# Christovis/astrild

Hardware: AMD Instinct MI355X
Metric: particles/sec CIC+3D-FFT P(k) on 1024^3 grid (higher is better)
Workload: dtype f32

## Files before the change

astrild_amd/csrc/fft_tile.hip:

```cpp
#include "ast_common.h"
#include "fft_roots.h"
#include "lowk_sums.h"
#include "paint_tile_geom.h"
#include <algorithm>
#include <cmath>
#include <cstring>
#include <mutex>
#include <vector>

namespace {

__device__ constexpr float kCos32[16] = {
    1.0f, 0.9807852804032304f, 0.9238795325112867f, 0.8314696123025452f, 0.7071067811865476f,
    0.5555702330196023f, 0.38268343236508984f, 0.19509032201612833f, 0.0f, -0.1950903220161282f,
    -0.3826834323650897f, -0.555570233019602f, -0.7071067811865475f, -0.8314696123025453f,
    -0.9238795325112867f, -0.9807852804032304f};
__device__ constexpr float kSin32[16] = {
    0.0f, 0.19509032201612825f, 0.3826834323650898f, 0.5555702330196022f, 0.7071067811865475f,
    0.8314696123025452f, 0.9238795325112867f, 0.9807852804032304f, 1.0f, 0.9807852804032304f,
    0.9238795325112867f, 0.8314696123025455f, 0.7071067811865476f, 0.5555702330196022f,
    0.3826834323650899f, 0.1950903220161286f};

typedef float f2v __attribute__((ext_vector_type(2)));
template <bool NT>
// ... 29 lines not shown
                v[blk + j] = a + b;
                const cf2 d = a - b;
                const int t = j * (16 / h);
                if (t == 0) v[blk + j + h] = d;
                else if (t == 8) v[blk + j + h] = d.yx * cf2{1.0f, -1.0f};
                else v[blk + j + h] = cmul_cf(d, cf2{kCos32[t], -kSin32[t]});
            }
        }
    }
#pragma unroll
    for (int i = 0; i < R; ++i) vv[i] = from_cf(v[i]);
}

__device__ inline int tile_isqrt(int v) {
    return (int)__builtin_amdgcn_sqrtf((float)v + 0.5f);
}

__global__ void tile_isqrt_table_kernel(int* out, int count) {
    for (int v = blockIdx.x * blockDim.x + threadIdx.x; v < count; v += gridDim.x * blockDim.x) out[v] = tile_isqrt(v);
}

struct ShellMask { const float2* src; long long lo2, hi2; int ky0 = 0; int pass = 0;
                   size_t src_elem_stride = 0, src_batch_stride = 0;
                   int epi_skip = 0, no_nyq = 0; };

constexpr int SHELL_BATCH = 8;
#ifndef XPASS_ATOMICS
#define XPASS_ATOMICS 1
#endif
struct ShellBatch { int count = 0; float2* work[SHELL_BATCH]; long long lo2[SHELL_BATCH], hi2[SHELL_BATCH]; };
struct C2RBatch { int count = 0; const float2* in[SHELL_BATCH]; float* out[SHELL_BATCH]; int kmax[SHELL_BATCH]; };

struct DiscEntry { int offb; unsigned S, cumS, lohi; };
struct PackDst { float2* out = nullptr; unsigned c1_log2 = 0; unsigned nbatch = 0; float2* self_out = nullptr; unsigned self_part = ~0u; unsigned pitch = 0;
                 const DiscEntry* disc = nullptr; const unsigned short* gk = nullptr; unsigned part = 0;
                 unsigned xmajor = 0; };

template <int R1, int R2, int C, bool POWER, bool INV = false, int PACK = 0, bool TAB = false>
__global__ void __launch_bounds__(C * (R1 > R2 ? R1 : R2))
__attribute__((amdgpu_waves_per_eu((POWER || C > 16) && R1 * R2 >= 1024 ? 4 : 1, (POWER || C > 16) && R1 * R2 >= 1024 ? 4 : 8)))
strided_c2c_kernel(float2* __restrict__ data, const float2* __restrict__ tw_g, size_t elem_stride,
                   size_t ncols, size_t batch_stride, unsigned tiles_per_batch, float scale,
                   double* __restrict__ partial, const unsigned* __restrict__ edge_fall, ShellMask mask = ShellMask{nullptr, 0, 0},
                   PackDst pack = PackDst{}, ShellBatch sb = ShellBatch{}) {
    constexpr int N = R1 * R2;
    constexpr int NT = C * (R1 > R2 ? R1 : R2);
    constexpr int NB = N / 2 - 1;
    constexpr bool SPLIT = (POWER || C > 16) && R1 == R2 && N * C * sizeof(float2) > 64 * 1024;
    constexpr int YN = SPLIT ? N / 2 : N;
    extern __shared__ float2 lds[];
    float2* Y = lds;
    float2* tw = lds + YN * C;
    double* shell = reinterpret_cast<double*>(lds + YN * C + N);
    unsigned tile = blockIdx.x % tiles_per_batch, b = blockIdx.x / tiles_per_batch;
    if ((gridDim.x / tiles_per_batch) % 8u == 0u) {
        const unsigned xcd = blockIdx.x & 7u, slot = blockIdx.x >> 3;
        b = (slot / tiles_per_batch) * 8u + xcd;
        tile = slot % tiles_per_batch;
    }
    const size_t c0 = (size_t)tile * C;
    if (INV && sb.count > 0) {
        data = sb.work[blockIdx.y];
        mask.lo2 = sb.lo2[blockIdx.y];
        mask.hi2 = sb.hi2[blockIdx.y];
    }
    if (INV && mask.hi2 > 0) {
        const long long kb = (long long)((int)b > N / 2 ? (int)b - N : (int)b);
        const long long r2 = (long long)(c0 * c0) + (mask.pass == 0 ? kb * kb : 0);
        if (r2 >= mask.hi2) return;
    }
    const float2* disc_base = nullptr;
    unsigned disc_S = 0;
    int disc_ky = 0;
    if (!INV && POWER && pack.disc != nullptr) {
        const unsigned subb = b % R1, gk = pack.gk[pack.part * (pack.nbatch / R1) + b / R1];
        const DiscEntry e = pack.disc[(size_t)tile * R2 + gk];
        const unsigned lo = e.lohi & 255u, hi = (e.lohi >> 8) & 255u;
        if (subb - lo >= hi - lo) {
            for (int i = threadIdx.x; i < NB; i += NT) partial[((size_t)b * tiles_per_batch + tile) * NB + i] = 0.0;
            return;
        }
        disc_ky = (int)(gk * R1 + subb);
        if (pack.xmajor) {
            disc_base = data + ((long long)e.offb + (long long)(subb * 16u)) * (long long)pack.xmajor;
            disc_S = 16u;
        } else {
            disc_base = data + ((long long)e.offb + (long long)(subb * 16u));
            disc_S = e.S;
        }
    } else if (!INV && POWER && (mask.hi2 > 0 || mask.no_nyq)) {
        const long long kyi = (long long)b + mask.ky0, ky = kyi > N / 2 ? kyi - N : kyi;
        if ((mask.hi2 > 0 && ky * ky + (long long)(c0 * c0) > mask.hi2) || (mask.no_nyq && c0 >= (size_t)(N / 2))) {
            for (int i = threadIdx.x; i < NB; i += NT) partial[((size_t)b * tiles_per_batch + tile) * NB + i] = 0.0;
            return;
        }
    }
    for (int i = threadIdx.x; i < N; i += NT) tw[i] = tw_g[i];
    if (POWER)
        for (int i = threadIdx.x; i <= NB; i += NT) shell[i] = 0.0;
    const int c = threadIdx.x % C, sub = threadIdx.x / C;
    const bool col_ok = (unsigned)c0 + (unsigned)c < (unsigned)ncols;
    float2 u[R2];
    {
        const bool task1 = sub < R2;
        float2 v[R1];
        const bool own = INV && mask.src != nullptr && mask.src_elem_stride != 0;
        size_t es_in = own ? mask.src_elem_stride : elem_stride;
        const float2* ubase = (INV && mask.src ? mask.src : data) + (size_t)b * (own ? mask.src_batch_stride : batch_stride);
        const int lsub = task1 ? sub : R2 - 1;
        uint32_t voff = (uint32_t)lsub * (uint32_t)es_in + min((uint32_t)c0 + (uint32_t)c, (uint32_t)ncols - 1u);
        if (POWER && !INV && disc_base != nullptr) {
            es_in = disc_S;
            ubase = disc_base;
            voff = (uint32_t)lsub * disc_S + (uint32_t)c;
        }
        if (INV && mask.hi2 > 0 && mask.pass == 1) {
            const long long c02 = (long long)(c0 * c0);
#pragma unroll
            for (int n1 = 0; n1 < R1; ++n1) {
                const int row = n1 * R2 + lsub;
                const long long ky = row > N / 2 ? row - N : row;
                v[n1] = make_float2(0.f, 0.f);
                if (ky * ky + c02 < mask.hi2) v[n1] = (ubase + (size_t)(n1 * R2) * es_in)[voff];
            }
        } else if (INV && mask.hi2 > 0) {
            const long long kyb = (long long)((int)b > N / 2 ? (int)b - N : (int)b);
            const long long r2yz = kyb * kyb + (long long)(c0 * c0);
#pragma unroll
            for (int n1 = 0; n1 < R1; ++n1) {
                const int lo = n1 * R2, hi = lo + R2 - 1;
                const long long kxmin = hi <= N / 2 ? lo : (lo >= N / 2 ? N - hi : 0);
                v[n1] = make_float2(0.f, 0.f);
                if (kxmin * kxmin + r2yz < mask.hi2) v[n1] = (ubase + (size_t)(n1 * R2) * es_in)[voff];
            }
        } else {
#pragma unroll
            for (int n1 = 0; n1 < R1; ++n1) v[n1] = ld_stream<(!INV && N >= 1024)>(ubase + (size_t)(n1 * R2) * es_in + voff);
        }
        if (INV) {
            if (mask.hi2 > 0 && mask.pass == 0) {
                const long long kz = (long long)min(c0 + c, ncols - 1), ky = (long long)((int)b > N / 2 ? (int)b - N : (int)b);
                const long long m2yz = ky * ky + kz * kz;
#pragma unroll
                for (int n1 = 0; n1 < R1; ++n1) {
                    const int row = n1 * R2 + lsub;
                    const long long kx = row > N / 2 ? row - N : row, m2 = kx * kx + m2yz;
                    if (m2 < mask.lo2 || m2 >= mask.hi2) v[n1] = make_float2(0.f, 0.f);
                }
            }
#pragma unroll
            for (int n1 = 0; n1 < R1; ++n1) v[n1].y = -v[n1].y;
        }
        fft_reg<R1>(v);
        __syncthreads();
        if (!SPLIT) {
            if (task1) {
#pragma unroll
                for (int k1 = 0; k1 < R1; ++k1) {
                    float2 y = v[bitrev(k1, ilog2(R1))];
                    if (k1 != 0) y = cmul(y, tw[sub * k1]);
// ... 53 lines not shown
                const int offb = __builtin_amdgcn_readlane(ev.x, k2);
                const unsigned S = (unsigned)__builtin_amdgcn_readlane(ev.y, k2), cumS = (unsigned)__builtin_amdgcn_readlane(ev.z, k2);
                const unsigned lohi = (unsigned)__builtin_amdgcn_readlane(ev.w, k2);
                const unsigned lo = lohi & 255u, hi = (lohi >> 8) & 255u, part = lohi >> 16;
                if (pack.xmajor) {
                    float2* const ub = pack.self_out + ((long long)offb * (long long)pack.xmajor + (long long)(b * 16u));
                    if ((unsigned)sub - lo < hi - lo)
                        st_stream<(N >= 1024)>(ub + ((uint32_t)sub * 16u * pack.xmajor + (uint32_t)(threadIdx.x & 15u)), x);
                    continue;
                }
                float2* const ub = (part == pack.self_part ? pack.self_out : pack.out + (size_t)pack.nbatch * cumS)
                                   + ((size_t)b * S + (long long)offb);
                if ((unsigned)sub - lo < hi - lo) st_stream<(N >= 1024)>(ub + threadIdx.x, x);
            }
        } else if (ok_s && !POWER) {
            float2* const base = data + (size_t)b * batch_stride + c0 + cs;
            const int room = (!INV && mask.hi2 > 0) ? (int)mask.hi2 - (int)(c0 * c0) : 0x7fffffff;
            const int wsub0 = __builtin_amdgcn_readfirstlane((int)threadIdx.x) / C, wsub1 = wsub0 + 64 / C - 1;
#pragma unroll
            for (int k2 = 0; k2 < R2; ++k2) {
                float2 x = u[bitrev(k2, ilog2(R2))];
                x.x *= scale;
                x.y *= INV ? -scale : scale;
                if (!INV) {
                    const int aky = R1 * k2 >= N / 2 ? N - (wsub1 + R1 * k2) : wsub0 + R1 * k2;
                    if (aky * aky > room) continue;
                }
                if (PACK) {
                    const unsigned part = (unsigned)(R1 * k2) >> pack.c1_log2, r0 = (unsigned)(R1 * k2) & ((1u << pack.c1_log2) - 1u);
                    float2* const ub = part == pack.self_part
                        ? pack.self_out + ((((size_t)b) << pack.c1_log2) + r0) * pack.pitch
                        : pack.out + ((((size_t)part * pack.nbatch + b) << pack.c1_log2) + r0) * pack.pitch;
                    st_stream<(N >= 1024)>(ub + ((uint32_t)sub * pack.pitch + (uint32_t)c0 + (uint32_t)cs), x);
                } else {
                    st_stream<(!INV && N >= 1024)>(base + (size_t)(sub + R1 * k2) * elem_stride, x);
                }
            }
        }
    }
    int tid_e = (int)threadIdx.x;
    asm volatile("" : "+v"(tid_e));
    if (POWER && (unsigned)c0 + (unsigned)(tid_e % C) < (unsigned)ncols && sub < R1) {
        if (TAB) acc_tab += (tid_e % C) * (NB + 2);
        unsigned fallmask = 0;
        const int kyi = disc_base != nullptr ? disc_ky : (int)b + mask.ky0;
        if (edge_fall) fallmask = edge_fall[((size_t)(disc_base != nullptr ? (unsigned)disc_ky : b) * tiles_per_batch + tile) * NT + threadIdx.x];
        const int kz = (int)c0 + tid_e % C;
        const int ky = kyi > N / 2 ? kyi - N : kyi;
        const int m2yz = ky * ky + kz * kz;
        const float w = TAB ? 1.0f : ((kz > 0 && kz < N / 2) ? 2.0f : 1.0f);
        const int wsub0 = __builtin_amdgcn_readfirstlane(tid_e) / C, wsub1 = wsub0 + 64 / C - 1;
        const int kyw = __builtin_amdgcn_readfirstlane(ky);
        const int room = (!INV && mask.epi_skip && mask.hi2 > 0) ? (int)mask.hi2 - kyw * kyw - (int)(c0 * c0) : 0x7fffffff;
#if XPASS_ATOMICS == 0
        double dead = 0.0;
#endif
#pragma unroll
        for (int k2 = 0; k2 < R2; ++k2) {
            const int akx = R1 * k2 >= N / 2 ? N - (wsub1 + R1 * k2) : wsub0 + R1 * k2;
            if (akx * akx > room) continue;
            const float2 x = u[bitrev(k2, ilog2(R2))];
            const int row = sub + R1 * k2;
            const int kx = row > N / 2 ? row - N : row;
            int sh = tile_isqrt(kx * kx + m2yz);
            sh -= (int)((fallmask >> k2) & 1u);
#if XPASS_ATOMICS == 1
            if (sh >= 1 && sh <= NB) atomicAdd(&acc_tab[sh], (double)(fmaf(x.x, x.x, x.y * x.y) * w));
#elif XPASS_ATOMICS == 2
            if (sh >= 1 && sh <= NB) atomicAdd(&shell[(sh & (N / 2 - 64)) | (tid_e & 63)], (double)(fmaf(x.x, x.x, x.y * x.y) * w));
// ... 100 lines not shown
            e[j] = f[j] + f[j + 8];
        }
        double g[4], s[4];
#pragma unroll
        for (int j = 1; j < 4; ++j) { g[j] = d[j] - d[8 - j]; s[j] = d[j] + d[8 - j]; }
#pragma unroll
        for (int k = 1; k < 6; k += 2) {
            double xr = d[0], xi = (k & 2) ? d[4] : -d[4];
#pragma unroll
            for (int j = 1; j < 4; ++j) {
                xr = fma(g[j], kC16f[(j * k) % 16], xr);
                xi = fma(s[j], kS16f[(j * k) % 16], xi);
            }
            emit(k, xr, xi);
        }
        real_dft8_low5(e, er, ei);
#pragma unroll
        for (int m = 0; m < 4; ++m) emit(2 * m, er[m], ei[m]);
    }
}

struct SlabFold { int xb0 = 0, ntx = 0, row_lo = 0, row_hi = 0; bool ranges = false; };

template <int R1, int R2, int C, int FOLDW, bool LOWK = false>
__global__ void __launch_bounds__(C * R2)
__attribute__((amdgpu_waves_per_eu(LOWK ? 4 : 1, LOWK ? 4 : 8)))
rows_r2c_kernel(const float* __restrict__ in, float2* __restrict__ out, const float2* __restrict__ tw_g,
                size_t nrows, size_t in_pitch, size_t out_pitch, float scale, float mean,
                const float* __restrict__ rec, const double2* __restrict__ lowk_lane = nullptr,
                double* __restrict__ lowz = nullptr, SlabFold sf = SlabFold{}) {
    constexpr int M = R1 * R2, N = 2 * M;
    constexpr int NT = C * R2;
    constexpr int R2P = R2 + 1;
    constexpr int MP = M + 1;
    extern __shared__ float2 lds[];
    float2* Y = lds;
    float2* tw = lds + C * (R1 * R2P > MP ? R1 * R2P : MP);
    for (int i = threadIdx.x; i < N; i += NT) tw[i] = tw_g[i];

    const size_t row0 = (size_t)blockIdx.x * C;
    const int n2 = threadIdx.x % R2, r = threadIdx.x / R2;
    {
        const float2* zin = reinterpret_cast<const float2*>(in + min(row0 + r, nrows - 1) * in_pitch);
        float2 v[R1];
        const float* src[3];
        int ns = 0;
        if (FOLDW != 0) {
            constexpr int W = FOLDW != 0 ? FOLDW : 2;
            const int ng = (int)(2 * M);
            const size_t row = min(row0 + r, nrows - 1);
            if (sf.ntx == 0) {
                const int xb = sf.xb0 + (int)(row / ng), trow = xb / ast::TX;
                ns = !sf.ranges || (trow >= sf.row_lo && trow < sf.row_hi)
                         ? ast::halo_sources<float, W>(rec, xb, (int)(row % ng), ng, ng / ast::TX, ng / ast::TY, src) : 0;
            } else {
                const int xb = sf.xb0 + (int)(row / ng), trow = xb / ast::TX;
                ns = trow >= sf.row_lo && trow < sf.row_hi
                         ? ast::halo_sources<float, W>(rec, xb, (int)(row % ng), ng, sf.ntx, ng / ast::TY, src, false) : 0;
            }
        }
#pragma unroll
        for (int n1 = 0; n1 < R1; ++n1) v[n1] = ld_stream<(N >= 1024)>(zin + n1 * R2 + n2);
        if (FOLDW != 0 && ns > 0) {
            auto rec_ld = [&](int s, int n1) { return ld_stream<(N >= 1024)>(reinterpret_cast<const float2*>(src[s]) + n1 * R2 + n2); };
            if (ns == 1) {
#pragma unroll
                for (int n1 = 0; n1 < R1; ++n1) {
                    const float2 t = rec_ld(0, n1);
                    v[n1].x += t.x;
                    v[n1].y += t.y;
                }
            } else {
                float2 h[R1];
// ... 43 lines not shown
                });
            }
            const int lane = threadIdx.x & 63;
            auto level = [&](auto count_tag, int mask) {
                constexpr int COUNT = decltype(count_tag)::value;
                const bool upper = (lane & mask) != 0;
#pragma unroll
                for (int i = 0; i < COUNT / 2; ++i) {
                    const double keep = upper ? acc[i + COUNT / 2] : acc[i];
                    const double send = upper ? acc[i] : acc[i + COUNT / 2];
                    acc[i] = keep + __shfl_xor(send, mask, 64);
                }
            };
            constexpr int TOP = R2 / 2;
            level(std::integral_constant<int, 14>{}, TOP);
            acc[7] = 0.0;
            level(std::integral_constant<int, 8>{}, TOP / 2);
            level(std::integral_constant<int, 4>{}, TOP / 4);
            level(std::integral_constant<int, 2>{}, TOP / 8);
            if (R2 == 32) acc[0] += __shfl_xor(acc[0], 1, 64);
            constexpr int SH = R2 == 32 ? 1 : 0;
            const int sel = lane >> SH;
            const int sub = ((sel >> 2) & 1) * 4 + ((sel >> 1) & 1) * 2 + (sel & 1);
            if ((R2 == 16 || (lane & 1) == 0) && sub < 7 && row0 + r < nrows)
                lowz[(row0 + r) * (size_t)(2 * (MBOX_FWD + 1)) + ((sel >> 3) & 1) * 7 + sub] = acc[0];
        }
#pragma unroll
        for (int n1 = 0; n1 < R1; ++n1) {
            v[n1].x -= mean;
            v[n1].y -= mean;
        }
        fft_reg<R1>(v);
        __syncthreads();
#pragma unroll
        for (int k1 = 0; k1 < R1; ++k1) {
            float2 y = v[bitrev(k1, ilog2(R1))];
            if (k1 != 0) y = cmul(y, tw[2 * n2 * k1]);
            Y[(r * R1 + k1) * R2P + n2] = y;
        }
    }
    __syncthreads();
    float2 u[R2];
    const int k1 = threadIdx.x % R1, r2 = threadIdx.x / R1;
    const bool task2 = r2 < C;
    if (task2) {
#pragma unroll
        for (int j = 0; j < R2; ++j) u[j] = Y[(r2 * R1 + k1) * R2P + j];
        fft_reg<R2>(u);
    }
    __syncthreads();
    if (task2) {
#pragma unroll
        for (int k2 = 0; k2 < R2; ++k2) Y[r2 * MP + k1 + R1 * k2] = u[bitrev(k2, ilog2(R2))];
    }
    __syncthreads();
    for (int i = threadIdx.x; i < C * (M / 2 + 1); i += NT) {
        const int rr = i / (M / 2 + 1), k = i % (M / 2 + 1);
        if (row0 + rr >= nrows) continue;
        const float2 zk = Y[rr * MP + k];
        const float2 zm = Y[rr * MP + ((M - k) & (M - 1))];
        float2* orow = out + (row0 + rr) * out_pitch;
        if (k == 0) {
            orow[0] = make_float2((zk.x + zk.y) * scale, 0.f);
            orow[M] = make_float2((zk.x - zk.y) * scale, 0.f);
            continue;
        }
        const float2 e = make_float2(0.5f * (zk.x + zm.x), 0.5f * (zk.y - zm.y));
        const float2 o = make_float2(0.5f * (zk.x - zm.x), 0.5f * (zk.y + zm.y));
        const float2 w = tw[k];
        const float2 t = cmul(o, w);
        st_stream<(N >= 1024)>(orow + k, make_float2((e.x + t.y) * scale, (e.y - t.x) * scale));
        st_stream<(N >= 1024)>(orow + M - k, make_float2((e.x - t.y) * scale, (-e.y - t.x) * scale));
    }
}

template <int R1, int R2, int C>
__global__ void __launch_bounds__(C * R2)
rows_c2r_kernel(const float2* __restrict__ in, float* __restrict__ out, const float2* __restrict__ tw_g,
// ... 389 lines not shown
    std::mutex m;
    std::vector<std::pair<std::pair<int, int>, float2*>> tabs;
    float2* get(int n) {
        std::lock_guard<std::mutex> lock(m);
        int dev = 0;
        if (hipGetDevice(&dev) != hipSuccess) return nullptr;
        for (auto& t : tabs) if (t.first.first == dev && t.first.second == n) return t.second;
        std::vector<float2> h(n);
        for (int i = 0; i < n; ++i) {
            const double a = -2.0 * M_PI * (double)i / (double)n;
            h[i] = make_float2((float)std::cos(a), (float)std::sin(a));
        }
        float2* d = nullptr;
        if (hipMalloc(&d, n * sizeof(float2)) != hipSuccess) return nullptr;
        if (hipMemcpy(d, h.data(), n * sizeof(float2), hipMemcpyHostToDevice) != hipSuccess) return nullptr;
        tabs.push_back({{dev, n}, d});
        return d;
    }
} g_tw;

template <int R1, int R2, int C, bool POWER>
int launch_c2c(float2* data, const float2* tw, size_t elem_stride, size_t ncols, size_t batch, size_t batch_stride,
               float scale, double* partial, hipStream_t s, const unsigned* edge_fall = nullptr, int ky0 = 0, long long prune2 = 0,
               PackDst disc = PackDst{}, int epi_skip = 0, int no_nyq = 0, int tables = 0) {
    constexpr int N = R1 * R2, NT = C * (R1 > R2 ? R1 : R2);
    constexpr bool SPLIT = (POWER || C > 16) && R1 == R2 && N * C * sizeof(float2) > 64 * 1024;
    const size_t lds = (size_t)((SPLIT ? N / 2 : N) * C + N) * sizeof(float2) + (POWER ? (N / 2) * sizeof(double) : 0);
    static ast::PerDeviceOnce attr_once;
    if (attr_once.need()) {
        AST_CHECK_HIP(hipFuncSetAttribute(reinterpret_cast<const void*>(&strided_c2c_kernel<R1, R2, C, POWER>),
                                          hipFuncAttributeMaxDynamicSharedMemorySize, (int)lds));
        if (POWER) AST_CHECK_HIP(hipFuncSetAttribute(reinterpret_cast<const void*>(&strided_c2c_kernel<R1, R2, C, POWER, false, 0, POWER>),
                                                     hipFuncAttributeMaxDynamicSharedMemorySize, (int)lds));
        attr_once.mark();
    }
    const size_t tiles = (ncols + C - 1) / C;
    AST_CHECK_ARG(tiles * batch < 0x7fffffffull);
    AST_CHECK_ARG((size_t)(R2 - 1) * elem_stride + ncols < (1ull << 29));
    ShellMask mask{nullptr, 0, prune2, ky0};
    mask.epi_skip = epi_skip;
    mask.no_nyq = no_nyq;
    if (POWER && tables)
        strided_c2c_kernel<R1, R2, C, POWER, false, 0, POWER><<<(unsigned)(tiles * batch), NT, lds, s>>>(data, tw, elem_stride, ncols,
                                                                                                       batch_stride, (unsigned)tiles, scale,
                                                                                                       partial, edge_fall, mask, disc);
    else
        strided_c2c_kernel<R1, R2, C, POWER><<<(unsigned)(tiles * batch), NT, lds, s>>>(data, tw, elem_stride, ncols,
                                                                                       batch_stride, (unsigned)tiles, scale,
                                                                                       partial, edge_fall, mask, disc);
    AST_CHECK_LAUNCH();
    return AST_OK;
}

template <int R1, int R2, int C>
int launch_c2c_inv(float2* data, const float2* tw, size_t elem_stride, size_t ncols, size_t batch, size_t batch_stride,
                   float scale, ShellMask mask, hipStream_t s, ShellBatch sb = ShellBatch{}) {
    constexpr int N = R1 * R2, NT = C * (R1 > R2 ? R1 : R2);
    const size_t lds = (size_t)(N * C + N) * sizeof(float2);
    static ast::PerDeviceOnce attr_once;
    if (attr_once.need()) {
        AST_CHECK_HIP(hipFuncSetAttribute(reinterpret_cast<const void*>(&strided_c2c_kernel<R1, R2, C, false, true>),
                                          hipFuncAttributeMaxDynamicSharedMemorySize, (int)lds));
        attr_once.mark();
    }
// ... 18 lines not shown
                                          hipFuncAttributeMaxDynamicSharedMemorySize, (int)lds));
        attr_once.mark();
    }
    const size_t tiles = (ncols + C - 1) / C;
    AST_CHECK_ARG(tiles * batch < 0x7fffffffull);
    AST_CHECK_ARG((size_t)(R2 - 1) * elem_stride + ncols < (1ull << 29));
    strided_c2c_kernel<R1, R2, C, false, false, PACKM><<<(unsigned)(tiles * batch), NT, lds, s>>>(
        data, tw, elem_stride, ncols, batch_stride, (unsigned)tiles, scale, nullptr, nullptr, ShellMask{nullptr, 0, 0}, pack);
    AST_CHECK_LAUNCH();
    return AST_OK;
}

int dispatch_c2c_inv(size_t n, float2* d, const float2* tw, size_t elem_stride, size_t ncols, size_t batch, size_t batch_stride,
                     float scale, ShellMask mask, hipStream_t s, ShellBatch sb = ShellBatch{}) {
    if (n == 1024) return launch_c2c_inv<32, 32, 16>(d, tw, elem_stride, ncols, batch, batch_stride, scale, mask, s, sb);
    if (n == 512) return launch_c2c_inv<16, 32, 16>(d, tw, elem_stride, ncols, batch, batch_stride, scale, mask, s, sb);
    return launch_c2c_inv<16, 16, 16>(d, tw, elem_stride, ncols, batch, batch_stride, scale, mask, s, sb);
}

constexpr int FWD_C = 32;
template <bool POWER>
int dispatch_c2c(size_t n, float2* d, const float2* tw, size_t elem_stride, size_t ncols, size_t batch,
                 size_t batch_stride, float scale, double* partial, hipStream_t s, const unsigned* edge_fall = nullptr, int ky0 = 0,
                 long long prune2 = 0, PackDst disc = PackDst{}, int epi_skip = 0, int no_nyq = 0, int tables = 0) {
    if constexpr (!POWER) { if (n == 1024) return launch_c2c<32, 32, FWD_C, false>(d, tw, elem_stride, ncols, batch, batch_stride, scale, partial, s, edge_fall, ky0, prune2); }
    if (n == 1024) return launch_c2c<32, 32, 16, POWER>(d, tw, elem_stride, ncols, batch, batch_stride, scale, partial, s, edge_fall, ky0, prune2, disc, epi_skip, no_nyq, tables);
    if (n == 512) return launch_c2c<16, 32, 16, POWER>(d, tw, elem_stride, ncols, batch, batch_stride, scale, partial, s, edge_fall, ky0, prune2, disc, epi_skip, no_nyq, tables);
    return launch_c2c<16, 16, 16, POWER>(d, tw, elem_stride, ncols, batch, batch_stride, scale, partial, s, edge_fall, ky0, prune2, disc, epi_skip, no_nyq, tables);
}

template <int R1, int R2, int C, int FOLDW = 0, bool LOWK = false>
int launch_r2c(const float* in, float2* out, const float2* tw, size_t nrows, size_t in_pitch, size_t out_pitch,
               float scale, float mean, hipStream_t s, const float* rec = nullptr, const double2* lowk_lane = nullptr,
               double* lowz = nullptr, SlabFold sf = SlabFold{}) {
    constexpr int M = R1 * R2, N = 2 * M, NT = C * R2;
    constexpr int BUF = C * (R1 * (R2 + 1) > M + 1 ? R1 * (R2 + 1) : M + 1);
    const size_t lds = (size_t)(BUF + N) * sizeof(float2);
    static ast::PerDeviceOnce attr_once;
    if (attr_once.need()) {
        AST_CHECK_HIP(hipFuncSetAttribute(reinterpret_cast<const void*>(&rows_r2c_kernel<R1, R2, C, FOLDW, LOWK>),
                                          hipFuncAttributeMaxDynamicSharedMemorySize, (int)lds));
        attr_once.mark();
    }
    const size_t blocks = (nrows + C - 1) / C;
    AST_CHECK_ARG(blocks < 0x7fffffffull);
    rows_r2c_kernel<R1, R2, C, FOLDW, LOWK><<<(unsigned)blocks, NT, lds, s>>>(in, out, tw, nrows, in_pitch, out_pitch, scale, mean, rec,
                                                                             lowk_lane, lowz, sf);
    AST_CHECK_LAUNCH();
    return AST_OK;
}

template <int R1, int R2, int C>
int launch_c2r(const float2* in, float* out, const float2* tw, size_t nrows, size_t in_pitch, size_t out_pitch, float scale,
               int kmax, hipStream_t s, C2RBatch cb = C2RBatch{}) {
    constexpr int M = R1 * R2, N = 2 * M, NT = C * R2;
    constexpr int BUF = C * (R1 * (R2 + 1) > M + 1 ? R1 * (R2 + 1) : M + 1);
    const size_t lds = (size_t)(BUF + N) * sizeof(float2);
    static ast::PerDeviceOnce attr_once;
    if (attr_once.need()) {
        AST_CHECK_HIP(hipFuncSetAttribute(reinterpret_cast<const void*>(&rows_c2r_kernel<R1, R2, C>),
                                          hipFuncAttributeMaxDynamicSharedMemorySize, (int)lds));
        attr_once.mark();
    }
    const size_t blocks = (nrows + C - 1) / C;
    AST_CHECK_ARG(blocks < 0x7fffffffull);
    rows_c2r_kernel<R1, R2, C><<<dim3((unsigned)blocks, (unsigned)(cb.count > 0 ? cb.count : 1)), NT, lds, s>>>(in, out, tw, nrows, in_pitch, out_pitch,
                                                                                                        scale, kmax, cb);
    AST_CHECK_LAUNCH();
    return AST_OK;
}
// ... 147 lines not shown
    out[i] = make_double2(cs, sn);
}
struct LowkLaneCache {
    std::mutex m;
    struct E { int dev, n; double2* d; };
    std::vector<E> tabs;
    const double2* get(int n, hipStream_t s) {
        std::lock_guard<std::mutex> lock(m);
        int dev = 0;
        if (hipGetDevice(&dev) != hipSuccess) return nullptr;
        for (auto& t : tabs) if (t.dev == dev && t.n == n) return t.d;
        const int lanes = n == 1024 ? 32 : 16;
        double2* d = nullptr;
        if (hipMalloc(&d, (size_t)lanes * 7 * 2 * sizeof(double2)) != hipSuccess) return nullptr;
        lowk_lane_kernel<<<2, 256, 0, s>>>(d, n, lanes);
        if (hipGetLastError() != hipSuccess || hipStreamSynchronize(s) != hipSuccess) { (void)hipFree(d); return nullptr; }
        tabs.push_back({dev, n, d});
        return d;
    }
} g_lowk_lane;

static int rows_r2c_impl(const void* in, void* out, int dtype, size_t n, size_t nrows, size_t in_pitch,
                         size_t out_pitch, double scale, double mean, void* stream, const void* rec = nullptr,
                         int window = 0, double* lowz = nullptr, SlabFold sf = SlabFold{}) {
    AST_CHECK_ARG(in != nullptr && out != nullptr && in != out && nrows >= 1);
    AST_CHECK_ARG(ast_fft_tile_supported(dtype, n));
    AST_CHECK_ARG(in_pitch >= n && in_pitch % 2 == 0 && out_pitch >= n / 2 + 1);
    AST_CHECK_ARG(((uintptr_t)in & 7) == 0 && ((uintptr_t)rec & 7) == 0 && ((uintptr_t)out & 7) == 0);
    const float2* tw = g_tw.get((int)n);
    if (!tw) { ast::set_error("ast_fft_tile_rows_r2c: twiddle table allocation failed"); return AST_ERR_HIP; }
    hipStream_t s = ast::as_stream(stream);
    AST_PROF("fft_tile.rows_r2c", s);
    const float* i = (const float*)in;
    float2* o = (float2*)out;
    if (lowz != nullptr) {
        const double2* lane = g_lowk_lane.get((int)n, s);
        if (!lane) { ast::set_error("ast_fft_tile_rows_r2c: low-k lane table allocation failed"); return AST_ERR_HIP; }
        const float* h = (const float*)rec;
        const float sc = (float)scale, mn = (float)mean;
        AST_CHECK_ARG(rec == nullptr || ((nrows == n * n || sf.ranges) && in_pitch == n && (window == AST_WIN_CIC || window == AST_WIN_TSC)));
        auto go = [&](auto r1, auto r2) {
            constexpr int R1 = decltype(r1)::value, R2 = decltype(r2)::value;
            if (rec == nullptr) return launch_r2c<R1, R2, 16, 0, true>(i, o, tw, nrows, in_pitch, out_pitch, sc, mn, s, nullptr, lane, lowz);
            if (window == AST_WIN_CIC) return launch_r2c<R1, R2, 16, 2, true>(i, o, tw, nrows, in_pitch, out_pitch, sc, mn, s, h, lane, lowz, sf);
            return launch_r2c<R1, R2, 16, 3, true>(i, o, tw, nrows, in_pitch, out_pitch, sc, mn, s, h, lane, lowz, sf);
        };
        if (n == 1024) return go(std::integral_constant<int, 16>{}, std::integral_constant<int, 32>{});
        if (n == 512) return go(std::integral_constant<int, 16>{}, std::integral_constant<int, 16>{});
        return go(std::integral_constant<int, 8>{}, std::integral_constant<int, 16>{});
    }
    if (rec != nullptr) {
        AST_CHECK_ARG((nrows == n * n || sf.ranges) && in_pitch == n && (window == AST_WIN_CIC || window == AST_WIN_TSC));
        const float* h = (const float*)rec;
        const float sc = (float)scale, mn = (float)mean;
        if (window == AST_WIN_CIC) {
            if (n == 1024) return launch_r2c<16, 32, 16, 2>(i, o, tw, nrows, in_pitch, out_pitch, sc, mn, s, h, nullptr, nullptr, sf);
            if (n == 512) return launch_r2c<16, 16, 16, 2>(i, o, tw, nrows, in_pitch, out_pitch, sc, mn, s, h, nullptr, nullptr, sf);
// ... 160 lines not shown
    const bool disc_asked = !getenv("AST_FFT_NO_PRUNE") && disc_env != nullptr && (disc_env[0] == '1' || disc_env[0] == '2');
    const bool nyq_binned = kf_rule != 0.0 && ast::float64_edge_norm((int)(n / 2), 0, 0, (int)(n / 2), kf_rule) != (int)(n / 2);
    const bool no_nyq = !disc_asked && !nyq_binned && !getenv("AST_FFT_NYQ_COLUMN");
    const size_t tiles = (nz + 15) / 16;
    auto lowk_rest = [&]() -> int {
        AST_CHECK_HIP(hipEventRecord(side->in, s));
        AST_CHECK_HIP(hipStreamWaitEvent(side->side, side->in, 0));
        {
            AST_PROF("fft_tile.lowk", side->side);
            int rc = lowk_modes((const float*)grid, (const float*)rec, window, (int)n, 0, (int)n, 0, modes, work, side->side, z_fused);
            if (rc != AST_OK) return rc;
            const double ng = (double)n * (double)n * (double)n;
            lowk_shell_kernel<<<1, 256, 0, side->side>>>(modes, boxsize * boxsize * boxsize / (ng * ng), kf_rule, lowk_sums);
            AST_CHECK_LAUNCH();
        }
        AST_CHECK_HIP(hipEventRecord(side->done, side->side));
        return AST_OK;
    };
    if (lowk) {
        side = g_side.get(s);
        if (!side) { ast::set_error("ast_fft_tile_power_3d: side stream creation failed"); return AST_ERR_HIP; }
        if (!z_fused) { const int rc = lowk_rest(); if (rc != AST_OK) return rc; }
    }
    int rc = rows_r2c_impl(grid, spec, dtype, n, n * n, n, nzp, 1.0, mean, stream, rec, window,
                           z_fused ? reinterpret_cast<double*>(work) : nullptr);
    if (rc != AST_OK) return rc;
    if (z_fused) { rc = lowk_rest(); if (rc != AST_OK) return rc; }
    const long long prune2 = getenv("AST_FFT_NO_PRUNE") ? 0 : (long long)(n / 2) * (long long)(n / 2);
    const double inv_ng = 1.0 / ((double)n * (double)n * (double)n);
    const bool use_disc = disc_asked;
    const int epi_skip = prune2 != 0 && !getenv("AST_FFT_NO_EPI_SKIP");
    const int tables = !getenv("AST_FFT_SHELL_ATOMICS");
    const unsigned xmajor = use_disc && disc_env[0] == '2' ? (unsigned)n : 0u;
    if (use_disc) {
        const DiscLayout::Dev* dv = nullptr;
        const DiscLayout* L = g_disc.get(n, 1, true, &dv);
        if (!L) { ast::set_error("ast_fft_tile_power_3d: disc table allocation failed"); return AST_ERR_HIP; }
        {
            AST_PROF("fft_tile.c2c", s);
            PackDst pk;
            pk.nbatch = (unsigned)n;
            pk.disc = dv->tab;
            pk.self_out = disc;
            pk.self_part = 0;
            pk.xmajor = xmajor;
            if (n == 1024) rc = launch_c2c_pack<32, 32, 16, 2>(spec, tw, nzp, nz, n, n * nzp, 1.0f, pk, s);
            else if (n == 512) rc = launch_c2c_pack<16, 32, 16, 2>(spec, tw, nzp, nz, n, n * nzp, 1.0f, pk, s);
            else rc = launch_c2c_pack<16, 16, 16, 2>(spec, tw, nzp, nz, n, n * nzp, 1.0f, pk, s);
            if (rc != AST_OK) return rc;
        }
        AST_PROF("fft_tile.c2c_power", s);
        const unsigned* edge_fall = nullptr;
        if (kf_rule != 0.0) {
            edge_fall = g_edge.get(n, boxsize, s);
            if (!edge_fall) { ast::set_error("ast_fft_tile_power_3d: edge table allocation failed"); return AST_ERR_HIP; }
        }
        PackDst src;
        src.disc = dv->tab;
        src.gk = dv->gk;
        src.nbatch = (unsigned)n;
        src.xmajor = xmajor;
        rc = dispatch_c2c<true>(n, disc, tw, xmajor ? 16 : L->S[0], nz, n, 16, (float)inv_ng, partial, s, edge_fall, 0, 0, src);
        if (rc != AST_OK) return rc;
    } else {
        {
            AST_PROF("fft_tile.c2c", s);
            rc = dispatch_c2c<false>(n, spec, tw, nzp, no_nyq ? n / 2 : nz, n, n * nzp, 1.0f, nullptr, s, nullptr, 0, prune2);
            if (rc != AST_OK) return rc;
        }
        AST_PROF("fft_tile.c2c_power", s);
        const unsigned* edge_fall = nullptr;
        if (kf_rule != 0.0) {
            edge_fall = g_edge.get(n, boxsize, s);
            if (!edge_fall) { ast::set_error("ast_fft_tile_power_3d: edge table allocation failed"); return AST_ERR_HIP; }
        }
        rc = dispatch_c2c<true>(n, spec, tw, n * nzp, nz, n, nzp, (float)inv_ng, partial, s, edge_fall, 0, prune2, PackDst{}, epi_skip, no_nyq, tables);
        if (rc != AST_OK) return rc;
    }
    AST_PROF("fft_tile.shell_reduce", s);
    const int nb = (int)(n / 2 - 1);
    double* partial2 = (double*)scratch;
    shell_partials_stage1_kernel<<<REDUCE_ROWS, 256, 0, s>>>(partial, n * tiles, nb, partial2);
    shell_partials_stage2_kernel<<<(nb + 7) / 8, 256, 0, s>>>(partial2, nb, boxsize * boxsize * boxsize, lowk ? MLOW : 0, psum);
    if (lowk) {
        AST_CHECK_HIP(hipStreamWaitEvent(s, side->done, 0));
        lowk_patch_kernel<<<1, 64, 0, s>>>(lowk_sums, MLOW, psum);
    }
    AST_CHECK_LAUNCH();
    return AST_OK;
}

extern "C" size_t ast_lowk_work_bytes(size_t n, size_t nx) {
    return (nx * n * (MBOX + 1) + nx * (2 * MBOX + 1) * (MBOX + 1) + (size_t)LOWK_XPARTS * LOWK_MODES) * sizeof(double2);
}
extern "C" int ast_lowk_mode_count(void) { return (int)LOWK_MODES; }
extern "C" int ast_lowk_shell_count(void) { return MLOW; }

extern "C" int ast_lowk_modes(const void* planes, int dtype, size_t n, size_t x0, size_t nx, int accumulate, void* modes,
                              void* work, size_t work_bytes, void* stream) {
// ... 273 lines not shown
```

Measured before the change: 88.68 billion.

## Fuse first radix-16 y-FFT stage into the z r2c pass and split y pass

```diff
diff --git a/astrild_amd/csrc/fft_tile.hip b/astrild_amd/csrc/fft_tile.hip
--- a/astrild_amd/csrc/fft_tile.hip
+++ b/astrild_amd/csrc/fft_tile.hip
@@ -75,12 +75,19 @@
 
 struct ShellMask { const float2* src; long long lo2, hi2; int ky0 = 0; int pass = 0;
                    size_t src_elem_stride = 0, src_batch_stride = 0;
-                   int epi_skip = 0, no_nyq = 0; };
+                   int epi_skip = 0, no_nyq = 0;
+                   int ysh = 0; };
 
 constexpr int SHELL_BATCH = 8;
 #ifndef XPASS_ATOMICS
 #define XPASS_ATOMICS 1
 #endif
+#ifndef YSPLIT_C
+#define YSPLIT_C 32
+#endif
+#ifndef YSPLIT_EPI_PAIRS
+#define YSPLIT_EPI_PAIRS 0
+#endif
 struct ShellBatch { int count = 0; float2* work[SHELL_BATCH]; long long lo2[SHELL_BATCH], hi2[SHELL_BATCH]; };
 struct C2RBatch { int count = 0; const float2* in[SHELL_BATCH]; float* out[SHELL_BATCH]; int kmax[SHELL_BATCH]; };
 
@@ -89,7 +96,7 @@
                  const DiscEntry* disc = nullptr; const unsigned short* gk = nullptr; unsigned part = 0;
                  unsigned xmajor = 0; };
 
-template <int R1, int R2, int C, bool POWER, bool INV = false, int PACK = 0, bool TAB = false>
+template <int R1, int R2, int C, bool POWER, bool INV = false, int PACK = 0, bool TAB = false, int YS = 0>
 __global__ void __launch_bounds__(C * (R1 > R2 ? R1 : R2))
 __attribute__((amdgpu_waves_per_eu((POWER || C > 16) && R1 * R2 >= 1024 ? 4 : 1, (POWER || C > 16) && R1 * R2 >= 1024 ? 4 : 8)))
 strided_c2c_kernel(float2* __restrict__ data, const float2* __restrict__ tw_g, size_t elem_stride,
@@ -99,6 +106,8 @@
     constexpr int N = R1 * R2;
     constexpr int NT = C * (R1 > R2 ? R1 : R2);
     constexpr int NB = N / 2 - 1;
+    constexpr int SIDE = YS != 0 ? YS : N;
+    static_assert(YS == 0 || (YS == 16 * N && !POWER && !INV && PACK == 0), "y split: the remaining S-point forward pass");
     constexpr bool SPLIT = (POWER || C > 16) && R1 == R2 && N * C * sizeof(float2) > 64 * 1024;
     constexpr int YN = SPLIT ? N / 2 : N;
     extern __shared__ float2 lds[];
@@ -125,6 +134,7 @@
     const float2* disc_base = nullptr;
     unsigned disc_S = 0;
     int disc_ky = 0;
+    const unsigned bky = (!INV && POWER && mask.ysh != 0) ? (b >> mask.ysh) + ((b & ((1u << mask.ysh) - 1u)) << 4) : b;
     if (!INV && POWER && pack.disc != nullptr) {
         const unsigned subb = b % R1, gk = pack.gk[pack.part * (pack.nbatch / R1) + b / R1];
         const DiscEntry e = pack.disc[(size_t)tile * R2 + gk];
@@ -142,7 +152,7 @@
             disc_S = e.S;
         }
     } else if (!INV && POWER && (mask.hi2 > 0 || mask.no_nyq)) {
-        const long long kyi = (long long)b + mask.ky0, ky = kyi > N / 2 ? kyi - N : kyi;
+        const long long kyi = (long long)bky + mask.ky0, ky = kyi > N / 2 ? kyi - N : kyi;
         if ((mask.hi2 > 0 && ky * ky + (long long)(c0 * c0) > mask.hi2) || (mask.no_nyq && c0 >= (size_t)(N / 2))) {
             for (int i = threadIdx.x; i < NB; i += NT) partial[((size_t)b * tiles_per_batch + tile) * NB + i] = 0.0;
             return;
@@ -188,7 +198,7 @@
             }
         } else {
 #pragma unroll
-            for (int n1 = 0; n1 < R1; ++n1) v[n1] = ld_stream<(!INV && N >= 1024)>(ubase + (size_t)(n1 * R2) * es_in + voff);
+            for (int n1 = 0; n1 < R1; ++n1) v[n1] = ld_stream<(!INV && SIDE >= 1024)>(ubase + (size_t)(n1 * R2) * es_in + voff);
         }
         if (INV) {
             if (mask.hi2 > 0 && mask.pass == 0) {
@@ -288,6 +298,12 @@
                 float2 x = u[bitrev(k2, ilog2(R2))];
                 x.x *= scale;
                 x.y *= INV ? -scale : scale;
+                if (YS != 0) {
+                    const int kyn = (int)(b & 15u) + 16 * (sub + R1 * k2), ky = kyn > SIDE / 2 ? kyn - SIDE : kyn;
+                    if (ky * ky > room) continue;
+                    st_stream<(SIDE >= 1024)>(base + (size_t)(sub + R1 * k2) * elem_stride, x);
+                    continue;
+                }
                 if (!INV) {
                     const int aky = R1 * k2 >= N / 2 ? N - (wsub1 + R1 * k2) : wsub0 + R1 * k2;
                     if (aky * aky > room) continue;
@@ -309,8 +325,8 @@
     if (POWER && (unsigned)c0 + (unsigned)(tid_e % C) < (unsigned)ncols && sub < R1) {
         if (TAB) acc_tab += (tid_e % C) * (NB + 2);
         unsigned fallmask = 0;
-        const int kyi = disc_base != nullptr ? disc_ky : (int)b + mask.ky0;
-        if (edge_fall) fallmask = edge_fall[((size_t)(disc_base != nullptr ? (unsigned)disc_ky : b) * tiles_per_batch + tile) * NT + threadIdx.x];
+        const int kyi = disc_base != nullptr ? disc_ky : (int)bky + mask.ky0;
+        if (edge_fall) fallmask = edge_fall[((size_t)(disc_base != nullptr ? (unsigned)disc_ky : bky) * tiles_per_batch + tile) * NT + threadIdx.x];
         const int kz = (int)c0 + tid_e % C;
         const int ky = kyi > N / 2 ? kyi - N : kyi;
         const int m2yz = ky * ky + kz * kz;
@@ -457,33 +473,42 @@
 
 struct SlabFold { int xb0 = 0, ntx = 0, row_lo = 0, row_hi = 0; bool ranges = false; };
 
-template <int R1, int R2, int C, int FOLDW, bool LOWK = false>
+template <int S>
+__device__ inline unsigned ysplit_y2(unsigned blk) {
+    static_assert(S % 8 == 0, "eight workgroups to a rotation");
+    const unsigned i = blk % (unsigned)S;
+    return (i & ~7u) | ((i + (i >> 3)) & 7u);
+}
+
+template <int R1, int R2, int C, int FOLDW, bool LOWK = false, bool YS = false>
 __global__ void __launch_bounds__(C * R2)
 __attribute__((amdgpu_waves_per_eu(LOWK ? 4 : 1, LOWK ? 4 : 8)))
 rows_r2c_kernel(const float* __restrict__ in, float2* __restrict__ out, const float2* __restrict__ tw_g,
                 size_t nrows, size_t in_pitch, size_t out_pitch, float scale, float mean,
                 const float* __restrict__ rec, const double2* __restrict__ lowk_lane = nullptr,
-                double* __restrict__ lowz = nullptr, SlabFold sf = SlabFold{}) {
+                double* __restrict__ lowz = nullptr, SlabFold sf = SlabFold{}, int ycols = 0) {
     constexpr int M = R1 * R2, N = 2 * M;
     constexpr int NT = C * R2;
     constexpr int R2P = R2 + 1;
     constexpr int MP = M + 1;
+    static_assert(!YS || C == 16, "y split: the workgroup's rows are the inputs of one radix-16 stage");
+    constexpr size_t RS = YS ? N / 16 : 1;
     extern __shared__ float2 lds[];
     float2* Y = lds;
     float2* tw = lds + C * (R1 * R2P > MP ? R1 * R2P : MP);
     for (int i = threadIdx.x; i < N; i += NT) tw[i] = tw_g[i];
 
-    const size_t row0 = (size_t)blockIdx.x * C;
+    const size_t row0 = YS ? (size_t)(blockIdx.x / (unsigned)RS) * N + ysplit_y2<YS ? N / 16 : 8>(blockIdx.x) : (size_t)blockIdx.x * C;
     const int n2 = threadIdx.x % R2, r = threadIdx.x / R2;
     {
-        const float2* zin = reinterpret_cast<const float2*>(in + min(row0 + r, nrows - 1) * in_pitch);
+        const float2* zin = reinterpret_cast<const float2*>(in + min(row0 + r * RS, nrows - 1) * in_pitch);
         float2 v[R1];
         const float* src[3];
         int ns = 0;
         if (FOLDW != 0) {
             constexpr int W = FOLDW != 0 ? FOLDW : 2;
             const int ng = (int)(2 * M);
-            const size_t row = min(row0 + r, nrows - 1);
+            const size_t row = min(row0 + r * RS, nrows - 1);
             if (sf.ntx == 0) {
                 const int xb = sf.xb0 + (int)(row / ng), trow = xb / ast::TX;
                 ns = !sf.ranges || (trow >= sf.row_lo && trow < sf.row_hi)
@@ -573,8 +598,8 @@
             constexpr int SH = R2 == 32 ? 1 : 0;
             const int sel = lane >> SH;
             const int sub = ((sel >> 2) & 1) * 4 + ((sel >> 1) & 1) * 2 + (sel & 1);
-            if ((R2 == 16 || (lane & 1) == 0) && sub < 7 && row0 + r < nrows)
-                lowz[(row0 + r) * (size_t)(2 * (MBOX_FWD + 1)) + ((sel >> 3) & 1) * 7 + sub] = acc[0];
+            if ((R2 == 16 || (lane & 1) == 0) && sub < 7 && row0 + r * RS < nrows)
+                lowz[(row0 + r * RS) * (size_t)(2 * (MBOX_FWD + 1)) + ((sel >> 3) & 1) * 7 + sub] = acc[0];
         }
 #pragma unroll
         for (int n1 = 0; n1 < R1; ++n1) {
@@ -605,6 +630,65 @@
         for (int k2 = 0; k2 < R2; ++k2) Y[r2 * MP + k1 + R1 * k2] = u[bitrev(k2, ilog2(R2))];
     }
     __syncthreads();
+    if constexpr (YS) {
+        constexpr int S = N / 16;
+        const unsigned y2 = ysplit_y2<S>(blockIdx.x);
+        float2* const obase = out + ((size_t)(blockIdx.x / (unsigned)S) * N + y2) * out_pitch;
+        auto stage_y = [&](float2 (&x)[16], int k) __attribute__((always_inline)) {
+            fft_reg<16>(x);
+#pragma unroll
+            for (int k1 = 0; k1 < 16; ++k1) {
+                float2 a = x[bitrev(k1, 4)];
+                if (k1 != 0) a = cmul(a, tw_g[y2 * k1]);
+                float2* const ub = obase + (size_t)(k1 * S) * out_pitch;
+                st_stream<(N >= 1024)>(ub + (uint32_t)k, a);
+            }
+        };
+#if YSPLIT_EPI_PAIRS
+        static_assert(!YS || NT >= M, "a thread per column");
+        if (const int k = threadIdx.x; k <= M / 2) {
+            const float2 w = tw[k];
+            float2 xa[16], xb[16];
+#pragma unroll
+            for (int rr = 0; rr < 16; ++rr) {
+                const float2 zk = Y[rr * MP + k];
+                const float2 zm = Y[rr * MP + ((M - k) & (M - 1))];
+                const float2 e = make_float2(0.5f * (zk.x + zm.x), 0.5f * (zk.y - zm.y));
+                const float2 o = make_float2(0.5f * (zk.x - zm.x), 0.5f * (zk.y + zm.y));
+                const float2 t = cmul(o, w);
+                xa[rr] = make_float2((e.x + t.y) * scale, (e.y - t.x) * scale);
+                xb[rr] = make_float2((e.x - t.y) * scale, (-e.y - t.x) * scale);
+                if (k == 0) {
+                    xa[rr] = make_float2((zk.x + zk.y) * scale, 0.f);
+                    xb[rr] = make_float2((zk.x - zk.y) * scale, 0.f);
+                }
+            }
+            stage_y(xa, k);
+            if (k != M / 2 && M - k < ycols) stage_y(xb, M - k);
+        }
+#else
+        static_assert(!YS || NT >= M, "a thread per column");
+        auto column = [&](int k) __attribute__((always_inline)) {
+            const int ka = k & (M - 1), km = (M - k) & (M - 1);
+            const float2 w = tw[k];
+            float2 x[16];
+#pragma unroll
+            for (int rr = 0; rr < 16; ++rr) {
+                const float2 zk = Y[rr * MP + ka];
+                const float2 zm = Y[rr * MP + km];
+                const float2 e = make_float2(0.5f * (zk.x + zm.x), 0.5f * (zk.y - zm.y));
+                const float2 o = make_float2(0.5f * (zk.x - zm.x), 0.5f * (zk.y + zm.y));
+                const float2 t = cmul(o, w);
+                x[rr] = make_float2((e.x + t.y) * scale, (e.y - t.x) * scale);
+                if (ka == 0) x[rr] = make_float2((k == 0 ? zk.x + zk.y : zk.x - zk.y) * scale, 0.f);
+            }
+            stage_y(x, k);
+        };
+        if ((int)threadIdx.x < M) column((int)threadIdx.x);
+        if (ycols > M && threadIdx.x == 0) column(M);
+#endif
+        return;
+    }
     for (int i = threadIdx.x; i < C * (M / 2 + 1); i += NT) {
         const int rr = i / (M / 2 + 1), k = i % (M / 2 + 1);
         if (row0 + rr >= nrows) continue;
@@ -1040,7 +1124,7 @@
 template <int R1, int R2, int C, bool POWER>
 int launch_c2c(float2* data, const float2* tw, size_t elem_stride, size_t ncols, size_t batch, size_t batch_stride,
                float scale, double* partial, hipStream_t s, const unsigned* edge_fall = nullptr, int ky0 = 0, long long prune2 = 0,
-               PackDst disc = PackDst{}, int epi_skip = 0, int no_nyq = 0, int tables = 0) {
+               PackDst disc = PackDst{}, int epi_skip = 0, int no_nyq = 0, int tables = 0, int ysh = 0) {
     constexpr int N = R1 * R2, NT = C * (R1 > R2 ? R1 : R2);
     constexpr bool SPLIT = (POWER || C > 16) && R1 == R2 && N * C * sizeof(float2) > 64 * 1024;
     const size_t lds = (size_t)((SPLIT ? N / 2 : N) * C + N) * sizeof(float2) + (POWER ? (N / 2) * sizeof(double) : 0);
@@ -1058,6 +1142,7 @@
     ShellMask mask{nullptr, 0, prune2, ky0};
     mask.epi_skip = epi_skip;
     mask.no_nyq = no_nyq;
+    mask.ysh = ysh;
     if (POWER && tables)
         strided_c2c_kernel<R1, R2, C, POWER, false, 0, POWER><<<(unsigned)(tiles * batch), NT, lds, s>>>(data, tw, elem_stride, ncols,
                                                                                                        batch_stride, (unsigned)tiles, scale,
@@ -1122,30 +1207,44 @@
 template <bool POWER>
 int dispatch_c2c(size_t n, float2* d, const float2* tw, size_t elem_stride, size_t ncols, size_t batch,
                  size_t batch_stride, float scale, double* partial, hipStream_t s, const unsigned* edge_fall = nullptr, int ky0 = 0,
-                 long long prune2 = 0, PackDst disc = PackDst{}, int epi_skip = 0, int no_nyq = 0, int tables = 0) {
+                 long long prune2 = 0, PackDst disc = PackDst{}, int epi_skip = 0, int no_nyq = 0, int tables = 0, int ysh = 0) {
     if constexpr (!POWER) { if (n == 1024) return launch_c2c<32, 32, FWD_C, false>(d, tw, elem_stride, ncols, batch, batch_stride, scale, partial, s, edge_fall, ky0, prune2); }
-    if (n == 1024) return launch_c2c<32, 32, 16, POWER>(d, tw, elem_stride, ncols, batch, batch_stride, scale, partial, s, edge_fall, ky0, prune2, disc, epi_skip, no_nyq, tables);
-    if (n == 512) return launch_c2c<16, 32, 16, POWER>(d, tw, elem_stride, ncols, batch, batch_stride, scale, partial, s, edge_fall, ky0, prune2, disc, epi_skip, no_nyq, tables);
-    return launch_c2c<16, 16, 16, POWER>(d, tw, elem_stride, ncols, batch, batch_stride, scale, partial, s, edge_fall, ky0, prune2, disc, epi_skip, no_nyq, tables);
-}
-
-template <int R1, int R2, int C, int FOLDW = 0, bool LOWK = false>
+    if (n == 1024) return launch_c2c<32, 32, 16, POWER>(d, tw, elem_stride, ncols, batch, batch_stride, scale, partial, s, edge_fall, ky0, prune2, disc, epi_skip, no_nyq, tables, ysh);
+    if (n == 512) return launch_c2c<16, 32, 16, POWER>(d, tw, elem_stride, ncols, batch, batch_stride, scale, partial, s, edge_fall, ky0, prune2, disc, epi_skip, no_nyq, tables, ysh);
+    return launch_c2c<16, 16, 16, POWER>(d, tw, elem_stride, ncols, batch, batch_stride, scale, partial, s, edge_fall, ky0, prune2, disc, epi_skip, no_nyq, tables, ysh);
+}
+
+template <int R1, int R2, int C, int SIDE>
+int launch_c2c_ysplit(float2* data, const float2* tw, size_t pitch, size_t ncols, long long prune2, hipStream_t s) {
+    constexpr int S = R1 * R2, NT = C * (R1 > R2 ? R1 : R2);
+    static_assert(16 * S == SIDE, "one radix-16 stage was done by the z pass");
+    const size_t lds = (size_t)(S * C + S) * sizeof(float2);
+    const size_t tiles = (ncols + C - 1) / C, batch = (size_t)16 * SIDE;
+    AST_CHECK_ARG(tiles * batch < 0x7fffffffull);
+    AST_CHECK_ARG((size_t)(R2 - 1) * pitch + ncols < (1ull << 29));
+    strided_c2c_kernel<R1, R2, C, false, false, 0, false, SIDE><<<(unsigned)(tiles * batch), NT, lds, s>>>(
+        data, tw, pitch, ncols, (size_t)S * pitch, (unsigned)tiles, 1.0f, nullptr, nullptr, ShellMask{nullptr, 0, prune2});
+    AST_CHECK_LAUNCH();
+    return AST_OK;
+}
+
+template <int R1, int R2, int C, int FOLDW = 0, bool LOWK = false, bool YS = false>
 int launch_r2c(const float* in, float2* out, const float2* tw, size_t nrows, size_t in_pitch, size_t out_pitch,
                float scale, float mean, hipStream_t s, const float* rec = nullptr, const double2* lowk_lane = nullptr,
-               double* lowz = nullptr, SlabFold sf = SlabFold{}) {
+               double* lowz = nullptr, SlabFold sf = SlabFold{}, int ycols = 0) {
     constexpr int M = R1 * R2, N = 2 * M, NT = C * R2;
     constexpr int BUF = C * (R1 * (R2 + 1) > M + 1 ? R1 * (R2 + 1) : M + 1);
     const size_t lds = (size_t)(BUF + N) * sizeof(float2);
     static ast::PerDeviceOnce attr_once;
     if (attr_once.need()) {
-        AST_CHECK_HIP(hipFuncSetAttribute(reinterpret_cast<const void*>(&rows_r2c_kernel<R1, R2, C, FOLDW, LOWK>),
+        AST_CHECK_HIP(hipFuncSetAttribute(reinterpret_cast<const void*>(&rows_r2c_kernel<R1, R2, C, FOLDW, LOWK, YS>),
                                           hipFuncAttributeMaxDynamicSharedMemorySize, (int)lds));
         attr_once.mark();
     }
     const size_t blocks = (nrows + C - 1) / C;
     AST_CHECK_ARG(blocks < 0x7fffffffull);
-    rows_r2c_kernel<R1, R2, C, FOLDW, LOWK><<<(unsigned)blocks, NT, lds, s>>>(in, out, tw, nrows, in_pitch, out_pitch, scale, mean, rec,
-                                                                             lowk_lane, lowz, sf);
+    rows_r2c_kernel<R1, R2, C, FOLDW, LOWK, YS><<<(unsigned)blocks, NT, lds, s>>>(in, out, tw, nrows, in_pitch, out_pitch, scale, mean, rec,
+                                                                                 lowk_lane, lowz, sf, ycols);
     AST_CHECK_LAUNCH();
     return AST_OK;
 }
@@ -1339,7 +1438,7 @@
 
 static int rows_r2c_impl(const void* in, void* out, int dtype, size_t n, size_t nrows, size_t in_pitch,
                          size_t out_pitch, double scale, double mean, void* stream, const void* rec = nullptr,
-                         int window = 0, double* lowz = nullptr, SlabFold sf = SlabFold{}) {
+                         int window = 0, double* lowz = nullptr, SlabFold sf = SlabFold{}, int ycols = 0) {
     AST_CHECK_ARG(in != nullptr && out != nullptr && in != out && nrows >= 1);
     AST_CHECK_ARG(ast_fft_tile_supported(dtype, n));
     AST_CHECK_ARG(in_pitch >= n && in_pitch % 2 == 0 && out_pitch >= n / 2 + 1);
@@ -1350,6 +1449,28 @@
     AST_PROF("fft_tile.rows_r2c", s);
     const float* i = (const float*)in;
     float2* o = (float2*)out;
+    if (ycols != 0) {
+        AST_CHECK_ARG(nrows == n * n && in_pitch == n && !sf.ranges && (ycols == (int)(n / 2) || ycols == (int)(n / 2 + 1)));
+        AST_CHECK_ARG(rec == nullptr || window == AST_WIN_CIC || window == AST_WIN_TSC);
+        const double2* lane = lowz != nullptr ? g_lowk_lane.get((int)n, s) : nullptr;
+        if (lowz != nullptr && !lane) { ast::set_error("ast_fft_tile_rows_r2c: low-k lane table allocation failed"); return AST_ERR_HIP; }
+        const float* h = (const float*)rec;
+        const float sc = (float)scale, mn = (float)mean;
+        auto go = [&](auto r1, auto r2) {
+            constexpr int R1 = decltype(r1)::value, R2 = decltype(r2)::value;
+            auto fw = [&](auto foldw) {
+                constexpr int FW = decltype(foldw)::value;
+                if (lowz != nullptr) return launch_r2c<R1, R2, 16, FW, true, true>(i, o, tw, nrows, in_pitch, out_pitch, sc, mn, s, h, lane, lowz, sf, ycols);
+                return launch_r2c<R1, R2, 16, FW, false, true>(i, o, tw, nrows, in_pitch, out_pitch, sc, mn, s, h, nullptr, nullptr, sf, ycols);
+            };
+            if (rec == nullptr) return fw(std::integral_constant<int, 0>{});
+            if (window == AST_WIN_CIC) return fw(std::integral_constant<int, 2>{});
+            return fw(std::integral_constant<int, 3>{});
+        };
+        if (n == 1024) return go(std::integral_constant<int, 16>{}, std::integral_constant<int, 32>{});
+        if (n == 512) return go(std::integral_constant<int, 16>{}, std::integral_constant<int, 16>{});
+        return go(std::integral_constant<int, 8>{}, std::integral_constant<int, 16>{});
+    }
     if (lowz != nullptr) {
         const double2* lane = g_lowk_lane.get((int)n, s);
         if (!lane) { ast::set_error("ast_fft_tile_rows_r2c: low-k lane table allocation failed"); return AST_ERR_HIP; }
@@ -1556,8 +1677,13 @@
         if (!side) { ast::set_error("ast_fft_tile_power_3d: side stream creation failed"); return AST_ERR_HIP; }
         if (!z_fused) { const int rc = lowk_rest(); if (rc != AST_OK) return rc; }
     }
+    const char* ys_env = getenv("AST_FFT_YSPLIT");
+    const bool ysplit = !disc_asked && (ys_env != nullptr ? ys_env[0] == '1' : n == 1024);
+    int ysh = 0;
+    if (ysplit) for (size_t v = n / 16; v > 1; v >>= 1) ++ysh;
     int rc = rows_r2c_impl(grid, spec, dtype, n, n * n, n, nzp, 1.0, mean, stream, rec, window,
-                           z_fused ? reinterpret_cast<double*>(work) : nullptr);
+                           z_fused ? reinterpret_cast<double*>(work) : nullptr, SlabFold{},
+                           ysplit ? (int)(no_nyq ? n / 2 : nz) : 0);
     if (rc != AST_OK) return rc;
     if (z_fused) { rc = lowk_rest(); if (rc != AST_OK) return rc; }
     const long long prune2 = getenv("AST_FFT_NO_PRUNE") ? 0 : (long long)(n / 2) * (long long)(n / 2);
@@ -1599,7 +1725,15 @@
     } else {
         {
             AST_PROF("fft_tile.c2c", s);
-            rc = dispatch_c2c<false>(n, spec, tw, nzp, no_nyq ? n / 2 : nz, n, n * nzp, 1.0f, nullptr, s, nullptr, 0, prune2);
+            if (ysplit) {
+                const float2* tws = g_tw.get((int)(n / 16));
+                if (!tws) { ast::set_error("ast_fft_tile_power_3d: twiddle table allocation failed"); return AST_ERR_HIP; }
+                const size_t yc = no_nyq ? n / 2 : nz;
+                if (n == 1024) rc = launch_c2c_ysplit<8, 8, YSPLIT_C, 1024>(spec, tws, nzp, yc, prune2, s);
+                else if (n == 512) rc = launch_c2c_ysplit<4, 8, YSPLIT_C, 512>(spec, tws, nzp, yc, prune2, s);
+                else rc = launch_c2c_ysplit<4, 4, YSPLIT_C, 256>(spec, tws, nzp, yc, prune2, s);
+            } else
+                rc = dispatch_c2c<false>(n, spec, tw, nzp, no_nyq ? n / 2 : nz, n, n * nzp, 1.0f, nullptr, s, nullptr, 0, prune2);
             if (rc != AST_OK) return rc;
         }
         AST_PROF("fft_tile.c2c_power", s);
@@ -1608,7 +1742,7 @@
             edge_fall = g_edge.get(n, boxsize, s);
             if (!edge_fall) { ast::set_error("ast_fft_tile_power_3d: edge table allocation failed"); return AST_ERR_HIP; }
         }
-        rc = dispatch_c2c<true>(n, spec, tw, n * nzp, nz, n, nzp, (float)inv_ng, partial, s, edge_fall, 0, prune2, PackDst{}, epi_skip, no_nyq, tables);
+        rc = dispatch_c2c<true>(n, spec, tw, n * nzp, nz, n, nzp, (float)inv_ng, partial, s, edge_fall, 0, prune2, PackDst{}, epi_skip, no_nyq, tables, ysh);
         if (rc != AST_OK) return rc;
     }
     AST_PROF("fft_tile.shell_reduce", s);
```

After: 92.13 billion (median of 6 runs). 3.9% higher.
